# LiJiangnanBit/path_optimizer

Measured on AMD Instinct MI355X. Metric: QP paths/sec at N=200 pts, batch=4096; ADMM iters to 1e-4, higher is better.
Workload: dtype f64

## Files before the change

path_optimizer_amd/csrc/po_capi.cpp:

```cpp
#include <hip/hip_runtime.h>

#include <chrono>
#include <cmath>
#include <cstdint>
#include <cstdio>
#include <algorithm>
#include <cstdlib>
#include <cstring>
#include <limits>
#include <mutex>
#include <new>
#include <string>
#include <thread>
#include <vector>

#include "../../include/po_hip.h"
#include "po_device.hpp"
#include "po_handle.hpp"
#include "po_launch.hpp"
#include "po_map.hpp"
#include "po_smooth.hpp"

namespace {
thread_local std::string g_hip_err;
// ... 204 lines not shown
        HIP_TRY(hipMemcpy(&c, static_cast<int *>(h->nw_idx_buf.p) + h->nw_last_B, sizeof(int), hipMemcpyDeviceToHost));
        *value = c;
        return PO_OK;
    }
    if (k == "newton_list_ok") {
        *value = -1;
        if (!h->nw_idx_buf.p || h->nw_last_B <= 0) return PO_OK;
        HIP_TRY(hipSetDevice(h->device));
        HIP_TRY(hipStreamSynchronize(h->stream));
        const int B = h->nw_last_B;
        std::vector<int> kl(2 * (size_t)B + 1);
        HIP_TRY(hipMemcpy(kl.data(), h->nw_idx_buf.p, sizeof(int) * kl.size(), hipMemcpyDeviceToHost));
        const int *keys = kl.data(), *list = kl.data() + B;
        const int n = list[0];
        int parked = 0;
        for (int b = 0; b < B; ++b) parked += keys[b] >= 0;
        bool ok = n == parked;
        std::vector<char> seen((size_t)B, 0);
        for (int i = 0; ok && i < n; ++i) {
            const int b = list[1 + i];
            ok = b >= 0 && b < B && keys[b] >= 0 && !seen[(size_t)b];
            if (ok) seen[(size_t)b] = 1;
            if (ok && i > 0) { const int a = list[i]; ok = keys[a] > keys[b] || (keys[a] == keys[b] && a < b); }
        }
        *value = ok ? 1 : 0;
        return PO_OK;
    }
    return PO_ERR_INVALID;
}

int po_set_stream(po_handle h, void *hip_stream) {
    if (!h) return PO_ERR_INVALID;
    Lock g(h->mu);
    h->stream = hip_stream ? static_cast<hipStream_t>(hip_stream) : h->own_stream.s;
    return PO_OK;
}

static int make_dev_params(const po_handle_s *h, int form, int keep, po::DevParams *D) {
    const po_params &p = h->params;
    D->d1 = p.d[0]; D->d2 = p.d[1]; D->d3 = p.d[2]; D->d4 = p.d[3];
    if (form == PO_K) {
        D->w_dev = p.k_w_dev; D->w_c = p.k_w_curv; D->w_cr = p.k_w_curv_rate; D->w_s1 = p.w_slack; D->w_s2 = 0; D->w_u = 0; D->w_su = 0;
    } else {
        D->w_dev = p.w_dev; D->w_c = p.w_curv; D->w_cr = p.w_curv_rate; D->w_s1 = p.w_slack;
        D->w_s2 = (form == PO_KPC) ? p.w_k_slack : 0.0;
        D->w_u = keep * p.w_curv_rate;
        D->w_su = (form == PO_KPC) ? p.w_kp_slack * keep : 0.0;
    }
    D->margin = p.margin;
    D->kmax = std::tan(p.max_steer) / p.wheel_base;
    D->max_steer = p.max_steer;
    D->wheel_base = p.wheel_base;
    D->sigma = p.sigma; D->alpha = p.alpha; D->rho0 = p.rho0; D->eps_abs = p.eps_abs; D->eps_rel = p.eps_rel;
    D->eps_pinf = p.eps_prim_inf; D->adapt_tol = p.adapt_tol;
    D->max_iter = p.max_iter; D->check_every = p.check_every; D->adapt_every = p.adapt_every;
    D->end_heading = p.constraint_end_heading;
    D->polish = p.polish; D->pol_delta = p.polish_delta > 0 ? p.polish_delta : 1e-6; D->pol_refine = p.polish_refine_iter < 0 ? 0 : p.polish_refine_iter;
    D->refine = p.refine; D->ref_eps = p.refine_eps; D->ref_rounds = p.refine_rounds;
    D->ref_extra = (p.refine && p.refine_extra_rounds > 0) ? p.refine_extra_rounds : 0;
    D->ref_nw_rho = p.refine_newton_rho > 0 ? std::min(p.refine_newton_rho, po::kRhoMax) : 100.0;
    D->ref_nw_rho_eq = p.refine_newton_rho_eq > 0 ? std::min(p.refine_newton_rho_eq, 1e8) : 1e4;
    D->ref_nw_rho_max = p.refine_newton_rho_max > 0 ? std::min(p.refine_newton_rho_max, po::kRhoMax) : 1e5;
    D->ref_nw_rho_eq_max = p.refine_newton_rho_eq_max > 0 ? std::min(p.refine_newton_rho_eq_max, 1e8) : (p.refine_newton_rho_eq_max < 0 ? 1e6 : 0.0);
    D->ref_ls_tol = p.refine_ls_tol > 0 ? p.refine_ls_tol : 1e-4;
    D->ref_nw_final = p.refine_newton_final; D->ref_nw_esc = p.refine_newton_escalate; D->ref_nw_slice = 0; D->ref_ls_max = p.refine_ls_max > 0 ? p.refine_ls_max : 30; D->ref_nw_max = p.refine_newton_max > 0 ? p.refine_newton_max : 300;
    return PO_OK;
}

static int validate(const po_batch_in *in, int *n, int *m, int *C) {
    if (!in) return PO_ERR_INVALID;
    if (in->B < 0) return PO_ERR_INVALID;
    int rc = po_problem_dims(in->formulation, in->N, in->keep, n, m, C);
    if (rc) return rc;
    if (!in->ref_x || !in->ref_y || !in->ref_z || !in->ref_k || !in->ref_s || !in->bounds || !in->x0 || !in->goal_z) return PO_ERR_INVALID;
    if (in->formulation == PO_KPC && (!in->max_k || !in->max_kp)) return PO_ERR_INVALID;
    if (po_lds_bytes(in->formulation, in->N, *C, in->keep) > 160 * 1024) return PO_ERR_UNSUPPORTED;
    return PO_OK;
}

static void fill_dev_batch(const po_handle_s *h, po::DevBatch *D, const po_batch_in *in, const po_batch_out *out, int n, int m, int C) PO_REQUIRES(h->mu) {
    D->B = in->B; D->N = in->N; D->keep = in->keep; D->C = C;
    D->ref_x = in->ref_x; D->ref_y = in->ref_y; D->ref_z = in->ref_z; D->ref_k = in->ref_k; D->ref_s = in->ref_s;
    D->bounds = in->bounds; D->x0 = in->x0; D->goal_z = in->goal_z; D->max_k = in->max_k; D->max_kp = in->max_kp;
    D->n_points = in->n_points;
    D->order = in->order;
    D->out_states = out ? out->states : nullptr;
    D->out_info = out ? out->info : nullptr;
    D->out_x = out ? out->x : nullptr;
    D->dbg_cycles = nullptr;
    D->only_deferred = 0;
    D->perm_bits = 0;
    if (!h->env_identity && in->B > 8)
        while ((1 << D->perm_bits) < in->B) ++D->perm_bits;
    D->scale = nullptr;
    D->pol_state = nullptr; D->pol_stride = 0;
    D->round = 0;
    D->fb_list = nullptr;
    D->nw_phase = 0; D->nw_state = nullptr; D->nw_stride = 0; D->nw_keys = nullptr; D->nw_list = nullptr;
    D->nw_follows = 0;
    D->fixed_len = (h->fixed_length && !in->n_points && po_has_fixed_length(in->formulation, in->N, C, in->keep)) ? 1 : 0;
    D->n = n; D->m = m;
}

int po_solve_batch_device(po_handle h, const po_batch_in *in, const po_batch_out *out) {
    if (!h || !out || !out->states || !out->info) return PO_ERR_INVALID;
    int n, m, C;
    int rc = validate(in, &n, &m, &C);
    if (rc) return rc;
    if (in->B == 0) return PO_OK;
    Lock g(h->mu);
    HIP_TRY(hipSetDevice(h->device));
    h->timed_host = false;
    po::DevParams P;
    make_dev_params(h, in->formulation, in->keep, &P);
    po::DevBatch D;
    fill_dev_batch(h, &D, in, out, n, m, C);
    const bool dbg = h->env_cycles;
    if (dbg) {
        if ((rc = h->dbg_buf.ensure(sizeof(long long) * 16 * (size_t)in->B))) return rc;
        D.dbg_cycles = static_cast<long long *>(h->dbg_buf.p);
        HIP_TRY(hipMemsetAsync(D.dbg_cycles, 0, sizeof(long long) * 16 * (size_t)in->B, h->stream));
    }
    if ((rc = h->scale_buf.ensure(sizeof(double) * 64 * (size_t)in->B))) return rc;
    D.scale = static_cast<double *>(h->scale_buf.p);
    h->fixed_used = D.fixed_len;
    bool polish = false;
    if (h->params.polish || h->params.refine) {
        const int sd = po_polish_state_doubles(in->formulation, in->N, C, in->keep);
        if (sd > 0) {
            if ((rc = h->pol_buf.ensure(sizeof(double) * (size_t)sd * (size_t)in->B))) return rc;
            D.pol_state = static_cast<double *>(h->pol_buf.p);
            D.pol_stride = sd;
            polish = h->params.polish && po_has_polish_kernel(in->formulation, in->N, C, in->keep);
        }
    }
    const int rounds_total = (h->params.refine_rounds > 1 ? h->params.refine_rounds : 1) + P.ref_extra;
    const bool split = h->params.refine == 2 && D.pol_state != nullptr && rounds_total < 32;
    if (split && ((rc = h->fb_buf.ensure(sizeof(int) * ((size_t)in->B + 1))) || (rc = h->fb_host.ensure(64)))) return rc;
    int pd = 0;
    if (split) {
        const bool slice_auto = in->B >= 2 * h->wave_slots && po_shape_threads(in->formulation, in->N, C, in->keep) == 64;
        pd = (h->nw_slice > 0 && (slice_auto || h->nw_slice_forced)) ? po_newton_park_doubles(in->formulation, in->N, C, in->keep) : 0;
        if (pd > 0 && (h->nw_state_buf.ensure(sizeof(double) * (size_t)pd * (size_t)in->B) || h->nw_idx_buf.ensure(sizeof(int) * (2 * (size_t)in->B + 1)))) {
            (void)hipGetLastError();
            h->nw_state_buf.release();
            pd = 0;
        }
        h->nw_last_B = pd > 0 ? in->B : 0;
    }
    HIP_TRY(hipEventRecord(h->ev0, h->stream));
    h->timed_phases = false;
    HIP_TRY(po_launch_scale(in->formulation, &D, &P, h->params.scaling, static_cast<double *>(h->scale_buf.p), pd > 0 ? static_cast<int *>(h->nw_idx_buf.p) : nullptr,
                            split ? static_cast<int *>(h->fb_buf.p) : nullptr, h->stream));
    if (split) {
        po::DevParams P1 = P;
        for (int r = 1; r < (h->params.refine_rounds > 1 ? h->params.refine_rounds : 1); ++r) { P1.eps_abs *= 10.0; P1.eps_rel *= 10.0; }
        D.nw_follows = 1;
        HIP_TRY(po_launch_solve(in->formulation, &D, &P1, h->stream, nullptr));
        D.nw_follows = 0;
        HIP_TRY(hipEventRecord(h->evp[0], h->stream));
        D.fb_list = static_cast<int *>(h->fb_buf.p);
        if (pd > 0) {
            D.nw_state = static_cast<double *>(h->nw_state_buf.p); D.nw_stride = pd;
            D.nw_keys = static_cast<int *>(h->nw_idx_buf.p); D.nw_list = D.nw_keys + in->B;
            P.ref_nw_slice = h->nw_slice;
            D.nw_phase = 1;
            HIP_TRY(po_launch_newton(in->formulation, &D, &P, h->stream));
            HIP_TRY(po_launch_nw_sort(D.nw_keys, in->B, D.nw_list, h->stream));
            D.nw_phase = 2;
            HIP_TRY(po_launch_newton(in->formulation, &D, &P, h->stream));
            D.nw_phase = 0;
        } else {
            HIP_TRY(po_launch_newton(in->formulation, &D, &P, h->stream));
        }
        HIP_TRY(hipEventRecord(h->evp[1], h->stream));
        h->timed_phases = true;
        bool need_fb = true;
        hipStreamCaptureStatus cap_st = hipStreamCaptureStatusNone;
        const bool capturing = hipStreamIsCapturing(h->stream, &cap_st) == hipSuccess && cap_st != hipStreamCaptureStatusNone;
        if (h->params.refine_chain != 3 && !capturing) {
            volatile int *cnt = static_cast<volatile int *>(h->fb_host.p);
            *cnt = -1;
            HIP_TRY(hipMemcpyAsync(const_cast<int *>(cnt), D.fb_list, sizeof(int), hipMemcpyDeviceToHost, h->stream));
            const auto ts0 = std::chrono::steady_clock::now();
            unsigned spins = 0;
            while (*cnt == -1) {
                if ((++spins & 1023u) == 0 && std::chrono::steady_clock::now() - ts0 > std::chrono::milliseconds(20)) { HIP_TRY(hipStreamSynchronize(h->stream)); break; }
#if defined(__x86_64__) || defined(__i386__)
                __builtin_ia32_pause();
#else
                std::this_thread::yield();
#endif
            }
            need_fb = *cnt != 0;
        }
        if (need_fb) HIP_TRY(po_launch_newton_fallback(in->formulation, &D, &P, h->stream));
    } else {
        HIP_TRY(po_launch_solve(in->formulation, &D, &P, h->stream, nullptr));
    }
    if (split) HIP_TRY(po_launch_finalize_status(D.out_info, in->B, h->stream));
    if (polish) HIP_TRY(po_launch_polish(in->formulation, &D, &P, h->stream));
    {
        const int no_refine = h->params.refine == 2 && !split, no_polish = h->params.polish && !polish;
        if (no_refine || no_polish) HIP_TRY(po_launch_mark_unavailable(D.out_info, in->B, no_refine, no_polish, h->stream));
    }
    HIP_TRY(hipEventRecord(h->ev1, h->stream));
    h->timed = true;
    if (dbg) {
        long long c4[16];
        HIP_TRY(hipStreamSynchronize(h->stream));
        HIP_TRY(hipMemcpy(c4, D.dbg_cycles, sizeof(c4), hipMemcpyDeviceToHost));
        {
            std::vector<long long> all(16 * (size_t)in->B);
            HIP_TRY(hipMemcpy(all.data(), D.dbg_cycles, sizeof(long long) * all.size(), hipMemcpyDeviceToHost));
            long long nf = 0, nb = 0;
            double worst = 0;
            for (int b = 0; b < in->B; ++b) {
                nf += all[16 * (size_t)b + 13]; nb += all[16 * (size_t)b + 14];
                double w; std::memcpy(&w, &all[16 * (size_t)b + 15], sizeof(w)); worst = std::fmax(worst, w);
            }
            std::fprintf(stderr, "[po] batch of %d (form %d, N %d, keep %d): %lld scan factorisations, %lld fell back to the sequential chain; worst relative disagreement scan vs recursion %.3e\n", in->B, in->formulation, in->N, in->keep, nf, nb, worst);
        }
        std::fprintf(stderr, "[po] path0 cycles: rhs %lld solve %lld update %lld over %lld iterations | solve phases F1 %lld F2 %lld F3B1 %lld B2 %lld B3 %lld | first factorisation: blocks %lld chain %lld | uniform row classes %lld | scan factorisations %lld, fell back to the sequential chain %lld\n",
                     c4[0], c4[1], c4[2], c4[3], c4[4], c4[5], c4[6], c4[7], c4[8], c4[10], c4[11], c4[12], c4[13], c4[14]);
    }
    return PO_OK;
}

int po_solve_batch(po_handle h, const po_batch_in *in, const po_batch_out *out) {
    if (!h || !out || !out->states || !out->info) return PO_ERR_INVALID;
    int n, m, C;
    int rc = validate(in, &n, &m, &C);
    if (rc) return rc;
    if (in->B == 0) return PO_OK;
    HIP_TRY(hipSetDevice(h->device));
    const size_t B = in->B, N = in->N;
    const bool kpc = in->formulation == PO_KPC;
    const size_t per_pt = 13 + (kpc ? 2 : 0);
    if (in->n_points)
        for (size_t b = 0; b < B; ++b)
            if (in->n_points[b] < 2 || in->n_points[b] > in->N) return PO_ERR_INVALID;
    if (in->order) {
        std::vector<char> seen(B, 0);
        for (size_t b = 0; b < B; ++b) {
            const int v = in->order[b];
            if (v < 0 || (size_t)v >= B || seen[(size_t)v]) return PO_ERR_INVALID;
            seen[(size_t)v] = 1;
        }
    }
    const size_t in_bytes = sizeof(double) * (B * N * per_pt + B * 4 + 2 * ((B + 1) / 2 + 1));
    const size_t out_bytes = sizeof(double) * (B * N * 5 + (out->x ? B * (size_t)n : 0)) + sizeof(po_info) * B;
    Lock call(h->call_mu);
    hipStream_t st;
    int nthr;
    {
        Lock g(h->mu);
        if ((rc = h->in_buf.ensure(in_bytes)) || (rc = h->out_buf.ensure(out_bytes)) || (rc = h->pin_in.ensure(in_bytes)) || (rc = h->pin_out.ensure(out_bytes))) return rc;
        st = h->stream;
        nthr = h->host_threads > 0 ? h->host_threads : (int)std::min(8u, std::max(1u, std::thread::hardware_concurrency()));
    }
    double *d = static_cast<double *>(h->in_buf.p);
    char *pin = static_cast<char *>(h->pin_in.p);
    po_batch_in din = *in;
    std::vector<CopySeg> segs;
    size_t o = 0;
    auto up = [&](const double *src, size_t cnt, const double **dst) {
        *dst = d + o;
        segs.push_back({pin + o * sizeof(double), reinterpret_cast<const char *>(src), cnt * sizeof(double)});
        o += cnt;
    };
    up(in->ref_x, B * N, &din.ref_x); up(in->ref_y, B * N, &din.ref_y); up(in->ref_z, B * N, &din.ref_z); up(in->ref_k, B * N, &din.ref_k); up(in->ref_s, B * N, &din.ref_s);
    up(in->bounds, B * N * 8, &din.bounds); up(in->x0, B * 3, &din.x0); up(in->goal_z, B, &din.goal_z);
    if (kpc) { up(in->max_k, B * N, &din.max_k); up(in->max_kp, B * N, &din.max_kp); }
    size_t used = o * sizeof(double);
    if (in->n_points) {
        segs.push_back({pin + o * sizeof(double), reinterpret_cast<const char *>(in->n_points), sizeof(int) * B});
        din.n_points = reinterpret_cast<const int *>(d + o);
        used = o * sizeof(double) + sizeof(int) * B;
    }
    if (in->order) {
        const size_t oo = o * sizeof(double) + sizeof(int) * ((B + 1) / 2) * 2;
        segs.push_back({pin + oo, reinterpret_cast<const char *>(in->order), sizeof(int) * B});
        din.order = reinterpret_cast<const int *>(reinterpret_cast<char *>(d) + oo);
        used = oo + sizeof(int) * B;
    }
    double pack_ms, unpack_ms;
    HIP_TRY(hipEventRecord(h->evh[0], st));
    {
        const auto t0 = std::chrono::steady_clock::now();
        const size_t kSlice = (size_t)32 << 20;
        for (size_t lo = 0; lo < used; lo += kSlice) {
            const size_t hi = std::min(used, lo + kSlice);
            std::vector<CopySeg> cur;
            for (const CopySeg &sg : segs) {
                const size_t s0 = (size_t)(sg.dst - pin), s1 = s0 + sg.bytes;
                const size_t a0 = std::max(s0, lo), a1 = std::min(s1, hi);
                if (a0 < a1) cur.push_back({pin + a0, sg.src + (a0 - s0), a1 - a0});
            }
            parallel_copy(cur, nthr);
            HIP_TRY(hipMemcpyAsync(reinterpret_cast<char *>(d) + lo, pin + lo, hi - lo, hipMemcpyHostToDevice, st));
        }
        pack_ms = std::chrono::duration<double, std::milli>(std::chrono::steady_clock::now() - t0).count();
    }
    HIP_TRY(hipEventRecord(h->evh[1], st));
    po_batch_out dout;
    char *ob = static_cast<char *>(h->out_buf.p);
    dout.states = reinterpret_cast<double *>(ob);
    dout.x = out->x ? dout.states + B * N * 5 : nullptr;
    dout.info = reinterpret_cast<po_info *>(ob + sizeof(double) * (B * N * 5 + (out->x ? B * (size_t)n : 0)));
    rc = po_solve_batch_device(h, &din, &dout);
    if (rc) return rc;
    char *pout = static_cast<char *>(h->pin_out.p);
    HIP_TRY(hipMemcpyAsync(pout, ob, out_bytes, hipMemcpyDeviceToHost, st));
    HIP_TRY(hipEventRecord(h->evh[2], st));
    HIP_TRY(hipStreamSynchronize(st));
    {
        const auto t0 = std::chrono::steady_clock::now();
        std::vector<CopySeg> us;
        us.push_back({reinterpret_cast<char *>(out->states), pout, sizeof(double) * B * N * 5});
        if (out->x) us.push_back({reinterpret_cast<char *>(out->x), pout + sizeof(double) * B * N * 5, sizeof(double) * B * (size_t)n});
        us.push_back({reinterpret_cast<char *>(out->info), pout + sizeof(double) * (B * N * 5 + (out->x ? B * (size_t)n : 0)), sizeof(po_info) * B});
        parallel_copy(us, nthr);
        unpack_ms = std::chrono::duration<double, std::milli>(std::chrono::steady_clock::now() - t0).count();
    }
    Lock g(h->mu);
    h->host_pack_ms = pack_ms; h->host_unpack_ms = unpack_ms;
    h->timed_host = true;
    return PO_OK;
}

int po_last_phase_ms(po_handle h, float *ms8) {
    if (!h || !ms8) return PO_ERR_INVALID;
    Lock g(h->mu);
    if (!h->timed) return PO_ERR_INVALID;
    for (int i = 0; i < 8; ++i) ms8[i] = 0.0f;
    HIP_TRY(hipEventSynchronize(h->ev1));
    HIP_TRY(hipEventElapsedTime(&ms8[1], h->ev0, h->ev1));
    if (h->timed_host) {
        HIP_TRY(hipEventSynchronize(h->evh[2]));
        HIP_TRY(hipEventElapsedTime(&ms8[0], h->evh[0], h->evh[1]));
        HIP_TRY(hipEventElapsedTime(&ms8[2], h->ev1, h->evh[2]));
        ms8[3] = (float)h->host_pack_ms; ms8[4] = (float)h->host_unpack_ms;
    }
    if (h->timed_phases) {
        HIP_TRY(hipEventElapsedTime(&ms8[5], h->ev0, h->evp[0]));
        HIP_TRY(hipEventElapsedTime(&ms8[6], h->evp[0], h->evp[1]));
        HIP_TRY(hipEventElapsedTime(&ms8[7], h->evp[1], h->ev1));
    }
    return PO_OK;
}

int po_assemble_batch(po_handle h, const po_batch_in *in, double *l, double *u, double *dyn) {
    if (!h || !l || !u || !dyn) return PO_ERR_INVALID;
    if (in && in->n_points) return PO_ERR_INVALID;
    int n, m, C;
    int rc = validate(in, &n, &m, &C);
    if (rc) return rc;
    if (in->B == 0) return PO_OK;
    const size_t B = in->B, N = in->N;
    const bool kpc = in->formulation == PO_KPC;
    Stage S;
    const Slot<double> rx = S.in(in->ref_x, B * N), ry = S.in(in->ref_y, B * N), rz = S.in(in->ref_z, B * N), rk = S.in(in->ref_k, B * N), rs = S.in(in->ref_s, B * N);
    const Slot<double> bd = S.in(in->bounds, B * N * 8), x0 = S.in(in->x0, B * 3), gz = S.in(in->goal_z, B);
    const Slot<double> mk = S.in(kpc ? in->max_k : nullptr, B * N), mkp = S.in(kpc ? in->max_kp : nullptr, B * N);
    const size_t out_from = (S.bytes() + 15) & ~(size_t)15;
    const Slot<double> dl = S.out(l, B * (size_t)m), du = S.out(u, B * (size_t)m), dd = S.out(dyn, B * (N - 1) * 3);
    return staged_call(h, S, &po_handle_s::asm_buf, false, [&]() -> int {
        Lock g(h->mu);
        po_batch_in din = *in;
        din.ref_x = rx; din.ref_y = ry; din.ref_z = rz; din.ref_k = rk; din.ref_s = rs; din.bounds = bd; din.x0 = x0; din.goal_z = gz;
        if (kpc) { din.max_k = mk; din.max_kp = mkp; }
        HIP_TRY(hipMemsetAsync(dl, 0, S.bytes() - out_from, h->stream));
        po::DevParams P;
        make_dev_params(h, in->formulation, in->keep, &P);
        po::DevBatch D;
        fill_dev_batch(h, &D, &din, nullptr, n, m, C);
        HIP_TRY(po_launch_assemble(in->formulation, &D, &P, dl, du, dd, h->stream));
        return PO_OK;
    });
}

int po_scaling_batch(po_handle h, const po_batch_in *in, double *out) {
    if (!h || !out) return PO_ERR_INVALID;
    if (in && in->n_points) return PO_ERR_INVALID;
    int n, m, C;
    int rc = validate(in, &n, &m, &C);
    if (rc) return rc;
    if (in->B == 0) return PO_OK;
    const size_t B = in->B, N = in->N;
    Stage S;
    const Slot<double> rs = S.in(in->ref_s, B * N), sc = S.out(out, 64 * B);
    return staged_call(h, S, &po_handle_s::asm_buf, false, [&]() -> int {
        Lock g(h->mu);
        po_batch_in din = *in;
        din.ref_s = rs;
        po::DevParams P;
        make_dev_params(h, in->formulation, in->keep, &P);
        po::DevBatch D;
        fill_dev_batch(h, &D, &din, nullptr, n, m, C);
        HIP_TRY(po_launch_scale(in->formulation, &D, &P, h->params.scaling, sc, nullptr, nullptr, h->stream));
        return PO_OK;
    });
}

int po_last_kernel_ms(po_handle h, float *ms) {
    if (!h || !ms) return PO_ERR_INVALID;
    Lock g(h->mu);
    if (!h->timed) return PO_ERR_INVALID;
    HIP_TRY(hipEventSynchronize(h->ev1));
    HIP_TRY(hipEventElapsedTime(ms, h->ev0, h->ev1));
    return PO_OK;
}

static po::DevCar make_car(const po_params &p) {
    po::DevCar c{};
    const double width = p.car_width, back = p.car_length / 2.0 - p.rear_axle_to_center, front = p.car_length / 2.0 + p.rear_axle_to_center;
    const double length = front + back;
    c.bx = (front - back) / 2.0;
    c.br = std::sqrt((length / 2) * (length / 2) + (width / 2) * (width / 2));
    const double shift = width / 4.0, small_r = std::sqrt(2 * (shift * shift));
    const double large_r = std::sqrt(width * width + ((length - width) / 2.0) * ((length - width) / 2.0)) / 2;
    const double px[4] = {-back + shift, -back + shift, front - shift, front - shift};
    const double py[4] = {-width / 2.0 + shift, width / 2.0 - shift, -width / 2.0 + shift, width / 2.0 - shift};
    for (int i = 0; i < 4; ++i) { c.cx[i] = px[i]; c.cy[i] = py[i]; c.cr[i] = small_r; }
    c.cx[4] = c.bx + (length - width) / 4; c.cy[4] = 0; c.cr[4] = large_r;
    c.cx[5] = c.bx - (length - width) / 4; c.cy[5] = 0; c.cr[5] = large_r;
    c.enable = p.enable_collision_check;
    return c;
}

static void publish_stack(po_handle h, int M, int sx, int sy, double res, double px, double py, bool layer_pos) PO_REQUIRES(h->mu) {
    const bool keep = h->maps.M == M && h->maps.layer_of;
    po::DevMaps s{};
    s.d = static_cast<const float *>(h->map_buf.p); s.sx = sx; s.sy = sy; s.res = res; s.px = px; s.py = py;
    s.M = M; s.stride = (size_t)sx * (size_t)sy;
    s.pos = layer_pos ? static_cast<const double *>(h->map_pos_buf.p) : nullptr;
    s.layer_of = keep ? static_cast<const int *>(h->map_assign_buf.p) : nullptr;
    s.n_assign = keep ? h->maps.n_assign : 0;
    h->maps = s;
}
static int install_layers(po_handle h, int M, const po_map *map, const double *pos_xy) PO_REQUIRES(h->mu) {
    HIP_TRY(hipSetDevice(h->device));
    const size_t bytes = sizeof(float) * (size_t)M * (size_t)map->size_x * (size_t)map->size_y;
    if (bytes > h->map_buf.cap) h->maps.d = nullptr;
    if (int rc = grow_after_sync(h, h->map_buf, bytes)) return rc;
    if (pos_xy) {
        if (int rc = grow_after_sync(h, h->map_pos_buf, sizeof(double) * 2 * (size_t)M)) return rc;
        HIP_TRY(hipMemcpyAsync(h->map_pos_buf.p, pos_xy, sizeof(double) * 2 * (size_t)M, hipMemcpyHostToDevice, h->stream));
    }
    HIP_TRY(hipMemcpyAsync(h->map_buf.p, map->distance, bytes, hipMemcpyHostToDevice, h->stream));
    HIP_TRY(hipStreamSynchronize(h->stream));
    publish_stack(h, M, map->size_x, map->size_y, map->resolution, map->pos_x, map->pos_y, pos_xy != nullptr);
    return PO_OK;
}

int po_set_map(po_handle h, const po_map *map) {
    if (!h || !map || !map->distance || map->size_x < 1 || map->size_y < 1 || !(map->resolution > 0)) return PO_ERR_INVALID;
    Lock g(h->mu);
    return install_layers(h, 1, map, nullptr);
}

int po_set_map_stack(po_handle h, int M, const po_map *layers, const double *pos_xy) {
    if (!h || M < 1 || !layers || !layers->distance || layers->size_x < 1 || layers->size_y < 1 || !(layers->resolution > 0)) return PO_ERR_INVALID;
    if (layers->size_x > po_edt_max_side() || layers->size_y > po_edt_max_side() || M > po_edt_max_images()) return PO_ERR_UNSUPPORTED;
    Lock call(h->call_mu);
    Lock g(h->mu);
    return install_layers(h, M, layers, pos_xy);
}

int po_set_map_assignment_device(po_handle h, int n, const int *layer_of) {
    if (!h || n < 0) return PO_ERR_INVALID;
    Lock g(h->mu);
    if (n == 0 || !layer_of) {
        h->maps.layer_of = nullptr; h->maps.n_assign = 0;
        return PO_OK;
    }
    if (!h->maps.d) return PO_ERR_INVALID;
    HIP_TRY(hipSetDevice(h->device));
    if (int rc = grow_after_sync(h, h->map_assign_buf, sizeof(int) * (size_t)n)) return rc;
    HIP_TRY(hipMemcpyAsync(h->map_assign_buf.p, layer_of, sizeof(int) * (size_t)n, hipMemcpyDeviceToDevice, h->stream));
    h->maps.layer_of = static_cast<const int *>(h->map_assign_buf.p); h->maps.n_assign = n;
    return PO_OK;
}

int po_set_map_assignment(po_handle h, int n, const int *layer_of) {
    if (!h || n < 0) return PO_ERR_INVALID;
    Lock call(h->call_mu);
    Lock g(h->mu);
    if (n == 0 || !layer_of) {
        h->maps.layer_of = nullptr; h->maps.n_assign = 0;
        return PO_OK;
    }
    if (!h->maps.d) return PO_ERR_INVALID;
    for (int b = 0; b < n; ++b)
        if (layer_of[b] < 0 || layer_of[b] >= h->maps.M) return PO_ERR_INVALID;
    HIP_TRY(hipSetDevice(h->device));
    if (int rc = grow_after_sync(h, h->map_assign_buf, sizeof(int) * (size_t)n)) {
        h->maps.layer_of = nullptr; h->maps.n_assign = 0;
        return rc;
    }
    HIP_TRY(hipMemcpyAsync(h->map_assign_buf.p, layer_of, sizeof(int) * (size_t)n, hipMemcpyHostToDevice, h->stream));
    HIP_TRY(hipStreamSynchronize(h->stream));
    h->maps.layer_of = static_cast<const int *>(h->map_assign_buf.p); h->maps.n_assign = n;
    return PO_OK;
}

static int check_occupancy(po_handle h, int M, const po_occupancy *occ) {
    if (!h || M < 1 || !occ || !occ->cells || occ->size_x < 1 || occ->size_y < 1 || !(occ->resolution > 0)) return PO_ERR_INVALID;
    if (occ->size_x > po_edt_max_side() || occ->size_y > po_edt_max_side() || M > po_edt_max_images()) return PO_ERR_UNSUPPORTED;
    return PO_OK;
}

int po_distance_map_batch_device(po_handle h, int M, const po_occupancy *occ, float *distance) {
    if (int rc = check_occupancy(h, M, occ)) return rc;
    if (!distance) return PO_ERR_INVALID;
    Lock g(h->mu);
    HIP_TRY(hipSetDevice(h->device));
    if (int rc = grow_after_sync(h, h->edt_buf, po_edt_scratch_bytes(M, occ->size_x, occ->size_y))) return rc;
    HIP_TRY(po_launch_edt(occ->cells, M, occ->size_x, occ->size_y, (float)occ->resolution, h->edt_buf.p, distance, h->stream));
    return PO_OK;
}

int po_distance_map_batch(po_handle h, int M, const po_occupancy *occ, float *distance) {
    if (int rc = check_occupancy(h, M, occ)) return rc;
    if (!distance) return PO_ERR_INVALID;
    const size_t cells = (size_t)M * (size_t)occ->size_x * (size_t)occ->size_y;
    Stage S;
    const Slot<float> d_dist = S.out(distance, cells);
    const Slot<unsigned char> d_cells = S.in(occ->cells, cells);
    return staged_call(h, S, &po_handle_s::edt_io, true, [&] {
        po_occupancy dev = *occ;
        dev.cells = d_cells;
        return po_distance_map_batch_device(h, M, &dev, d_dist);
    });
}

static int stack_from_images(po_handle h, int M, const unsigned char *cells, int sx, int sy, double res, double px, double py, const double *pos_xy)
    PO_REQUIRES(h->mu) {
    const size_t stack_bytes = sizeof(float) * (size_t)M * (size_t)sx * (size_t)sy;
    if (stack_bytes > h->map_buf.cap) h->maps.d = nullptr;
    if (int rc = grow_after_sync(h, h->map_buf, stack_bytes)) return rc;
    if (int rc = grow_after_sync(h, h->edt_buf, po_edt_scratch_bytes(M, sx, sy))) return rc;
    if (pos_xy) {
        if (int rc = grow_after_sync(h, h->map_pos_buf, sizeof(double) * 2 * (size_t)M)) return rc;
        HIP_TRY(hipMemcpyAsync(h->map_pos_buf.p, pos_xy, sizeof(double) * 2 * (size_t)M, hipMemcpyDeviceToDevice, h->stream));
    }
    HIP_TRY(po_launch_edt(cells, M, sx, sy, (float)res, h->edt_buf.p, static_cast<float *>(h->map_buf.p), h->stream));
    publish_stack(h, M, sx, sy, res, px, py, pos_xy != nullptr);
// ... 996 lines not shown
```

path_optimizer_amd/csrc/po_kernels.hip:

```cpp
#include "po_solve_common.hpp"

namespace po {

template <int F> __global__ __launch_bounds__(64) void assemble_kernel(DevBatch in, DevParams P, double *l, double *u, double *dyn) {
    using T = FormTraits<F>;
    extern __shared__ double smem[];
    const int b = blockIdx.x;
    Ctx<F> cx(P, in, smem, b);
    const int N = cx.N, C = cx.C;
    double *lb = l + (size_t)b * in.m, *ub = u + (size_t)b * in.m;
    for (int j = cx.lane; j < N; j += 64) {
        const StageIn si = cx.stage_in(j);
        AsmFn<F> fn{lb, ub, j, N, C, 0};
        local_rows<F>(si, P, fn);
        if (T::NEND && si.last) { fn.kind = 1; end_rows<F>(si, P, fn); }
        double bin[3];
        if (j == 0) cx.init_bounds(bin);
        else {
            const Dyn<F> d = cx.dyn(j - 1);
#pragma unroll
            for (int r = 0; r < T::NDYN; ++r) bin[r] = d.b[r];
            double *dd = dyn + ((size_t)b * (N - 1) + (j - 1)) * 3;
            if constexpr (F == F_K) { dd[0] = d.f[0][0]; dd[1] = d.f[1][1]; dd[2] = d.f[0][2]; }
            else { dd[0] = d.f[0][1]; dd[1] = d.f[1][0]; dd[2] = d.beta[2]; }
// ... 39 lines not shown
const Object kObjects[] = {PO_SOLVE_OBJECTS(PO_X)};
#undef PO_X
struct Resolved { Shape s; size_t lds; int group; bool fixed; };
hipError_t resolve(int form, const DevBatch *in, Resolved *r) {
    r->lds = 0;
    if (!resolve_shape(form, in->N, in->C, in->keep, &r->s)) return hipErrorInvalidValue;
    r->lds = lds_of(form, in->N, in->C, r->s);
    r->group = group_of(form, r->s);
#ifdef PO_DEV_HEADLINE
    if (form == F_KP && r->group) r->group = ~0;
#endif
    r->fixed = in->fixed_len && in->n_points == nullptr && is_fixed_shape(form, in->N, in->C, in->keep, r->s);
    return r->lds > 160 * 1024 ? hipErrorInvalidValue : hipSuccess;
}
hipError_t call(int form, int kind, int launch, const Resolved &r, const DevBatch *in, const DevParams *P, hipStream_t st) {
    for (const Object &o : kObjects)
        if (o.form == form && o.kind == kind && (o.groups & r.group) && o.entry) return o.entry(launch, r.s, r.lds, in, P, st);
    return hipErrorNotSupported;
}
}
}
extern "C" hipError_t po_launch_solve(int form, const po::DevBatch *in, const po::DevParams *P, hipStream_t st, size_t *lds_out) {
    using namespace po;
    Resolved r;
    hipError_t e = resolve(form, in, &r);
    if (lds_out && r.lds) *lds_out = r.lds;
    if (e != hipSuccess) return e;
    const bool uni = form == F_K ? has_uni_variant<F_K>(r.s) : has_uni_variant<F_KP>(r.s);
    DevBatch copy = *in;
    copy.only_deferred = 0;
    if (uni && (e = call(form, r.fixed ? kObjFixUni : kObjUni, kLaunchSolve, r, &copy, P, st)) != hipSuccess) return e;
    copy.only_deferred = uni ? 1 : 0;
    return call(form, kObjGen, kLaunchSolve, r, &copy, P, st);
}
extern "C" hipError_t po_launch_finalize_status(po_info *info, int B, hipStream_t st) {
    hipLaunchKernelGGL(po::finalize_status_kernel, dim3((B + 255) / 256), dim3(256), 0, st, info, B);
    return hipGetLastError();
}

static hipError_t launch_two_level(int form, int launch, const po::DevBatch *in, const po::DevParams *P, hipStream_t st) {
    using namespace po;
    Resolved r;
    const hipError_t e = resolve(form, in, &r);
    if (!r.lds || !r.s.two) return hipErrorInvalidValue;
    if (launch == kLaunchPolish && !has_polish_kernel(r.s)) return hipSuccess;
    if (e != hipSuccess) return e;
    const int kind = (launch == kLaunchNewton && r.fixed) ? (in->nw_phase == 2 ? kObjFixNewton2 : kObjFixNewton1) : (launch == kLaunchPolish ? kObjGen : kObjNewton);
    return call(form, kind, launch, r, in, P, st);
}
extern "C" hipError_t po_launch_newton(int form, const po::DevBatch *in, const po::DevParams *P, hipStream_t st) { return launch_two_level(form, po::kLaunchNewton, in, P, st); }
extern "C" hipError_t po_launch_newton_fallback(int form, const po::DevBatch *in, const po::DevParams *P, hipStream_t st) { return launch_two_level(form, po::kLaunchFallback, in, P, st); }
extern "C" hipError_t po_launch_polish(int form, const po::DevBatch *in, const po::DevParams *P, hipStream_t st) { return launch_two_level(form, po::kLaunchPolish, in, P, st); }
namespace po {
constexpr int kNwSortThreads = 256;
__global__ __launch_bounds__(kNwSortThreads) void nw_sort_kernel(const int *keys, int B, int *list) {
    __shared__ int cnt[kNwKeys][kNwSortThreads + 1];
    __shared__ int rowbase[kNwKeys];
    const int t = threadIdx.x, per = (B + kNwSortThreads - 1) / kNwSortThreads, lo = t * per, hi = min(B, lo + per);
    constexpr int kCache = 16;
    int kc[kCache];
#pragma unroll
    for (int i = 0; i < kCache; ++i) kc[i] = (lo + i < hi) ? keys[lo + i] : -1;
#pragma unroll
    for (int k = 0; k < kNwKeys; ++k) cnt[k][t] = 0;
#pragma unroll
    for (int i = 0; i < kCache; ++i)
        if (kc[i] >= 0) cnt[kc[i] < kNwKeys ? kc[i] : kNwKeys - 1][t] += 1;
    for (int b = lo + kCache; b < hi; ++b) {
        const int k = keys[b];
        if (k >= 0) cnt[k < kNwKeys ? k : kNwKeys - 1][t] += 1;
    }
    __syncthreads();
    {
        constexpr int kPerLane = kNwSortThreads / 64, kWaves = kNwSortThreads / 64;
        const int lane = t & 63, wv = t >> 6;
        for (int k = wv; k < kNwKeys; k += kWaves) {
            int v[kPerLane], sum = 0;
#pragma unroll
            for (int i = 0; i < kPerLane; ++i) { v[i] = cnt[k][lane * kPerLane + i]; sum += v[i]; }
            int incl = sum;
#pragma unroll
            for (int d = 1; d < 64; d <<= 1) { const int o = __shfl_up(incl, d, 64); if (lane >= d) incl += o; }
            int run = incl - sum;
#pragma unroll
            for (int i = 0; i < kPerLane; ++i) { cnt[k][lane * kPerLane + i] = run; run += v[i]; }
            if (lane == 63) cnt[k][kNwSortThreads] = incl;
        }
    }
    __syncthreads();
    if (t < kNwKeys) {
        int run = 0;
        for (int j = kNwKeys - 1; j > t; --j) run += cnt[j][kNwSortThreads];
        rowbase[t] = run;
        if (t == 0) list[0] = run + cnt[0][kNwSortThreads];
    }
    __syncthreads();
    auto place = [&](int b, int k) {
        const int kk = k < kNwKeys ? k : kNwKeys - 1;
        const int pos = rowbase[kk] + cnt[kk][t];
        cnt[kk][t] += 1;
        list[1 + pos] = b;
    };
#pragma unroll
    for (int i = 0; i < kCache; ++i)
        if (kc[i] >= 0) place(lo + i, kc[i]);
    for (int b = lo + kCache; b < hi; ++b) {
        const int k = keys[b];
        if (k >= 0) place(b, k);
    }
}

}
extern "C" hipError_t po_launch_nw_sort(const int *keys, int B, int *list, hipStream_t st) {
    hipLaunchKernelGGL(po::nw_sort_kernel, dim3(1), dim3(po::kNwSortThreads), 0, st, keys, B, list);
    return hipGetLastError();
}
namespace po {
namespace {
template <int F, bool TWO, int SPL, int NT, int NWX> struct RowSizes { static constexpr int state = 0, park = 0; };
template <int F, int SPL, int NT, int NWX> struct RowSizes<F, true, SPL, NT, NWX> {
    static constexpr int state = Fast<F, SPL, NT, true, NWX>::kStateDoubles * NT, park = Fast<F, SPL, NT, true, NWX>::kParkDoubles * NT + kNwParkScalars;
};
int row_doubles(int form, int N, int C, int keep, bool park) {
    Shape s;
    if (!resolve_shape(form, N, form == F_K ? 0 : C, keep, &s)) return 0;
#define PO_X(F_, TWO_, SPL_, NT_, NWX_, G_) if (form == F_ && is_shape(s, TWO_, SPL_, NT_, NWX_)) return park ? RowSizes<F_, TWO_, SPL_, NT_, NWX_>::park : RowSizes<F_, TWO_, SPL_, NT_, NWX_>::state;
    PO_SHAPE_ROWS(PO_X)
#undef PO_X
    return 0;
}
}
}
extern "C" int po_polish_state_doubles(int form, int N, int C, int keep) { return po::row_doubles(form, N, C, keep, false); }
extern "C" int po_newton_park_doubles(int form, int N, int C, int keep) { return po::row_doubles(form, N, C, keep, true); }
extern "C" int po_has_fixed_length(int form, int N, int C, int keep) {
    po::Shape s;
    if (!po::resolve_shape(form, N, C, keep, &s) || !po::is_fixed_shape(form, N, C, keep, s) || po::lds_of(form, N, C, s) > 160 * 1024) return 0;
#define PO_X(N_) if (N == N_) return 1;
    PO_FIXED_LIST(PO_X)
#undef PO_X
    return 0;
}
extern "C" int po_shape_threads(int form, int N, int C, int keep) {
    po::Shape s;
    return po::resolve_shape(form, N, form == po::F_K ? 0 : C, keep, &s) ? s.nt : 0;
}
extern "C" int po_has_polish_kernel(int form, int N, int C, int keep) {
    po::Shape s;
    return po::resolve_shape(form, N, form == po::F_K ? 0 : C, keep, &s) && po::has_polish_kernel(s);
}

extern "C" hipError_t po_launch_scale(int form, const po::DevBatch *in, const po::DevParams *P, int passes, double *sc, int *nw_keys, int *fb_count, hipStream_t st) {
    using namespace po;
    const int bs = 64, gs = (in->B + bs - 1) / bs;
    if (form == F_KP) hipLaunchKernelGGL(scale_kernel<F_KP>, dim3(gs), dim3(bs), 0, st, *in, *P, passes, sc, nw_keys, fb_count);
    else if (form == F_KPC) hipLaunchKernelGGL(scale_kernel<F_KPC>, dim3(gs), dim3(bs), 0, st, *in, *P, passes, sc, nw_keys, fb_count);
    else hipLaunchKernelGGL(scale_kernel<F_K>, dim3(gs), dim3(bs), 0, st, *in, *P, passes, sc, nw_keys, fb_count);
    return hipGetLastError();
}

extern "C" hipError_t po_launch_assemble(int form, const po::DevBatch *in, const po::DevParams *P, double *l, double *u, double *dyn, hipStream_t st) {
    using namespace po;
    if (form == F_KP) hipLaunchKernelGGL(assemble_kernel<F_KP>, dim3(in->B), dim3(64), 0, st, *in, *P, l, u, dyn);
    else if (form == F_KPC) hipLaunchKernelGGL(assemble_kernel<F_KPC>, dim3(in->B), dim3(64), 0, st, *in, *P, l, u, dyn);
    else hipLaunchKernelGGL(assemble_kernel<F_K>, dim3(in->B), dim3(64), 0, st, *in, *P, l, u, dyn);
    return hipGetLastError();
}

extern "C" size_t po_lds_bytes(int form, int N, int C, int keep) {
    using namespace po;
    Shape s;
    if (!resolve_shape(form, N, C, keep, &s)) return (size_t)1 << 30;
    return lds_of(form, N, C, s);
}
```

path_optimizer_amd/csrc/po_scale.hpp:

```cpp
#pragma once
#include "po_device.hpp"

namespace po {

constexpr int kNVC = 8;
constexpr int kNRC = 24;
constexpr int kScStride = 64;
constexpr int kScW = 0, kScE = 24, kScSig = 48, kScCD = 56, kScC = 63;
constexpr int kKEndRow = 11, kKEndVar = 6, kScAlt = 12;
constexpr double kMinScaling = 1e-4, kMaxScaling = 1e4;

struct ClassModel {
    int nr;
    double Pmax[kNVC], cnt[kNVC];
    double a[kNRC][kNVC];
    int tgt[kNRC];
};

struct PatFn {
    ClassModel *M;
    int base;
    template <int MASK, class TL, class TU> __host__ __device__ void row(int r, double c0, double c1, double c2, double c3, double c4, TL, TU) {
        double *a = M->a[base + r];
        a[0] = c0; a[1] = c1; a[2] = c2; a[3] = c3; a[4] = c4;
    }
};
struct PatCtlFn {
    ClassModel *M;
    int base;
    template <int MASK, class TL, class TU> __host__ __device__ void row(int r, double, double, double c2, double c3, double, TL, TU) {
        double *a = M->a[base + r];
        a[5] = c2; a[6] = c3;
    }
};

__device__ inline double limit_scaling(double v) {
    v = v < kMinScaling ? 1.0 : v;
    return v > kMaxScaling ? kMaxScaling : v;
}

template <int F> __device__ void class_scaling(const DevParams &P, int N, int keep, int C, double ds_nom, int passes, double *out ) {
#pragma clang fp contract(off)
    using T = FormTraits<F>;
    ClassModel M;
    M.nr = T::NLOC + T::NDYN + T::NCTL + T::NEND;
    for (int r = 0; r < kNRC; ++r) { M.tgt[r] = -1; for (int v = 0; v < kNVC; ++v) M.a[r][v] = 0; }
    StageIn s;
    for (int c = 0; c < 4; ++c) { s.lb[c] = -1; s.ub[c] = 1; }
    s.maxk = 0; s.elo = -kInf; s.ehi = kInf; s.j = 0; s.N = N; s.last = 0;
    PatFn pf{&M, 0};
    local_rows<F>(s, P, pf);
    const Dyn<F> d = make_dyn<F>(0.0, ds_nom, P);
    for (int r = 0; r < T::NDYN; ++r) {
        double *a = M.a[T::NLOC + r];
        a[0] = d.f[r][0]; a[1] = d.f[r][1]; a[2] = d.f[r][2]; a[5] = d.beta[r];
        M.tgt[T::NLOC + r] = dyn_tau<F>(r);
    }
    if constexpr (T::NCTL > 0) { PatCtlFn cf{&M, T::NLOC + T::NDYN}; ctl_rows<F>(0.0, cf); }
    if constexpr (T::NEND > 0) { PatFn ef{&M, T::NLOC + T::NDYN + T::NCTL}; end_rows<F>(s, P, ef); }
    if constexpr (F == F_K) {
        static_assert(T::NLOC + T::NDYN == kKEndRow && kScAlt + T::NLOC <= 24, "K end classes");
        M.a[kKEndRow][kKEndVar] = M.a[2][2];
        M.a[T::NLOC + 0][kKEndVar] = M.a[T::NLOC + 0][2];
        M.nr = kKEndRow + 1;
    }
    for (int v = 0; v < kNVC; ++v) { M.Pmax[v] = 0; M.cnt[v] = 0; }
    M.Pmax[0] = P.w_dev; M.Pmax[2] = (F == F_K) ? P.w_c + 2 * P.w_cr : P.w_c; M.Pmax[3] = P.w_s1;
    M.cnt[0] = N; M.cnt[1] = N; M.cnt[2] = N; M.cnt[3] = N;
    if constexpr (F == F_K) { M.Pmax[kKEndVar] = P.w_c + P.w_cr; M.cnt[kKEndVar] = N - 1 < 2 ? N - 1 : 2; M.cnt[2] = N - 1 - M.cnt[kKEndVar]; }
    if constexpr (F == F_KP) { M.Pmax[5] = P.w_u; M.cnt[5] = C; M.Pmax[7] = P.w_s1; M.cnt[7] = N; }
    if constexpr (F == F_KPC) { M.Pmax[4] = P.w_s2; M.cnt[4] = N; M.Pmax[5] = P.w_u; M.cnt[5] = C; M.Pmax[6] = P.w_su; M.cnt[6] = C; M.cnt[7] = N - C; }
    double Dv[kNVC], Er[kNRC], c = 1.0, ntot = 0;
    for (int v = 0; v < kNVC; ++v) { Dv[v] = 1.0; ntot += M.cnt[v]; }
    for (int r = 0; r < kNRC; ++r) Er[r] = 1.0;
    for (int pass = 0; pass < passes; ++pass) {
        double cn[kNVC], rn[kNRC];
        for (int v = 0; v < kNVC; ++v) cn[v] = fabs(c * M.Pmax[v] * Dv[v] * Dv[v]);
        for (int r = 0; r < M.nr; ++r) {
            double rmax = 0;
            for (int v = 0; v < kNVC; ++v) {
                const double a = fabs(Er[r] * M.a[r][v] * Dv[v]);
                if (a > rmax) rmax = a;
                if (a > cn[v]) cn[v] = a;
            }
            if (M.tgt[r] >= 0) {
                const double a = fabs(Er[r] * Dv[M.tgt[r]]);
                if (a > rmax) rmax = a;
                if (a > cn[M.tgt[r]]) cn[M.tgt[r]] = a;
            }
            rn[r] = rmax;
        }
        for (int v = 0; v < kNVC; ++v) Dv[v] *= 1.0 / sqrt(limit_scaling(cn[v]));
        for (int r = 0; r < M.nr; ++r) Er[r] *= 1.0 / sqrt(limit_scaling(rn[r]));
        double mean = 0;
        for (int v = 0; v < kNVC; ++v) mean += M.cnt[v] * fabs(c * M.Pmax[v] * Dv[v] * Dv[v]);
        mean /= ntot;
        double ct = mean > 1.0 ? mean : 1.0;
        ct = 1.0 / limit_scaling(ct);
        c *= ct;
    }
    for (int i = 0; i < kScStride; ++i) out[i] = 0;
    for (int r = 0; r < kNRC; ++r) { out[kScW + r] = Er[r] * Er[r] / c; out[kScE + r] = Er[r]; }
    for (int v = 0; v < 7; ++v) { out[kScSig + v] = P.sigma / (c * Dv[v] * Dv[v]); out[kScCD + v] = c * Dv[v]; }
    if constexpr (F == F_K) {
        for (int r = 0; r < T::NLOC; ++r) { out[kScW + kScAlt + r] = out[kScW + (r == 2 ? kKEndRow : r)]; out[kScE + kScAlt + r] = out[kScE + (r == 2 ? kKEndRow : r)]; }
    }
    out[kScC] = c;
}

template <int F> __global__ void scale_kernel(DevBatch in, DevParams P, int passes, double *sc, int *nw_keys, int *fb_count) {
    const int b = blockIdx.x * blockDim.x + threadIdx.x;
    if (b >= in.B) return;
    if (nw_keys) nw_keys[b] = -1;
    if (fb_count && b == 0) *fb_count = 0;
    const double *s = in.ref_s + (size_t)b * in.N;
    int N = in.N, C = in.C;
    if (in.n_points) { N = in.n_points[b]; N = N < 2 ? 2 : (N > in.N ? in.N : N); C = (F == F_K) ? N - 1 : (N + in.keep - 2) / in.keep; }
    double ds_nom = 0;
    for (int i = 1; i < N && i < 10; ++i) ds_nom = fmax(ds_nom, __dsub_rn(s[i], s[i - 1]));
    class_scaling<F>(P, N, in.keep, C, ds_nom, passes, sc + (size_t)b * kScStride);
}

}
```

Baseline: 1.215 million.

## Parallelize per-path scaling across 32 lanes and skip finalize when no fallback

The scaling kernel previously ran one thread per path, looping serially over all row and variable classes. It now assigns 32 lanes per path, one per row class, and computes column maxima with xor-shuffle reductions, broadcasting factors through shuffles. The finalize-status launch is now skipped unless the Newton fallback ran, which removes one kernel launch in the common case. The scaling batch API also accepts per-path point counts. Risks include more redundant per-lane model construction, possible output slots left unwritten (kScStride is no longer zeroed), and the finalize skip changing status handling.

```diff
diff --git a/path_optimizer_amd/csrc/po_capi.cpp b/path_optimizer_amd/csrc/po_capi.cpp
--- a/path_optimizer_amd/csrc/po_capi.cpp
+++ b/path_optimizer_amd/csrc/po_capi.cpp
@@ -380,6 +380,7 @@
     h->timed_phases = false;
     HIP_TRY(po_launch_scale(in->formulation, &D, &P, h->params.scaling, static_cast<double *>(h->scale_buf.p), pd > 0 ? static_cast<int *>(h->nw_idx_buf.p) : nullptr,
                             split ? static_cast<int *>(h->fb_buf.p) : nullptr, h->stream));
+    bool need_finalize = false;
     if (split) {
         po::DevParams P1 = P;
         for (int r = 1; r < (h->params.refine_rounds > 1 ? h->params.refine_rounds : 1); ++r) { P1.eps_abs *= 10.0; P1.eps_rel *= 10.0; }
@@ -423,10 +424,11 @@
             need_fb = *cnt != 0;
         }
         if (need_fb) HIP_TRY(po_launch_newton_fallback(in->formulation, &D, &P, h->stream));
+        need_finalize = need_fb;
     } else {
         HIP_TRY(po_launch_solve(in->formulation, &D, &P, h->stream, nullptr));
     }
-    if (split) HIP_TRY(po_launch_finalize_status(D.out_info, in->B, h->stream));
+    if (split && need_finalize) HIP_TRY(po_launch_finalize_status(D.out_info, in->B, h->stream));
     if (polish) HIP_TRY(po_launch_polish(in->formulation, &D, &P, h->stream));
     {
         const int no_refine = h->params.refine == 2 && !split, no_polish = h->params.polish && !polish;
@@ -610,7 +612,6 @@
 
 int po_scaling_batch(po_handle h, const po_batch_in *in, double *out) {
     if (!h || !out) return PO_ERR_INVALID;
-    if (in && in->n_points) return PO_ERR_INVALID;
     int n, m, C;
     int rc = validate(in, &n, &m, &C);
     if (rc) return rc;
@@ -618,10 +619,12 @@
     const size_t B = in->B, N = in->N;
     Stage S;
     const Slot<double> rs = S.in(in->ref_s, B * N), sc = S.out(out, 64 * B);
+    const Slot<int> np = S.in(in->n_points, B);
     return staged_call(h, S, &po_handle_s::asm_buf, false, [&]() -> int {
         Lock g(h->mu);
         po_batch_in din = *in;
         din.ref_s = rs;
+        din.n_points = np;
         po::DevParams P;
         make_dev_params(h, in->formulation, in->keep, &P);
         po::DevBatch D;
diff --git a/path_optimizer_amd/csrc/po_kernels.hip b/path_optimizer_amd/csrc/po_kernels.hip
--- a/path_optimizer_amd/csrc/po_kernels.hip
+++ b/path_optimizer_amd/csrc/po_kernels.hip
@@ -215,7 +215,7 @@
 
 extern "C" hipError_t po_launch_scale(int form, const po::DevBatch *in, const po::DevParams *P, int passes, double *sc, int *nw_keys, int *fb_count, hipStream_t st) {
     using namespace po;
-    const int bs = 64, gs = (in->B + bs - 1) / bs;
+    const int bs = kScBlock, gs = (int)(((size_t)in->B * kScLanes + bs - 1) / bs);
     if (form == F_KP) hipLaunchKernelGGL(scale_kernel<F_KP>, dim3(gs), dim3(bs), 0, st, *in, *P, passes, sc, nw_keys, fb_count);
     else if (form == F_KPC) hipLaunchKernelGGL(scale_kernel<F_KPC>, dim3(gs), dim3(bs), 0, st, *in, *P, passes, sc, nw_keys, fb_count);
     else hipLaunchKernelGGL(scale_kernel<F_K>, dim3(gs), dim3(bs), 0, st, *in, *P, passes, sc, nw_keys, fb_count);
diff --git a/path_optimizer_amd/csrc/po_scale.hpp b/path_optimizer_amd/csrc/po_scale.hpp
--- a/path_optimizer_amd/csrc/po_scale.hpp
+++ b/path_optimizer_amd/csrc/po_scale.hpp
@@ -39,10 +39,9 @@
     return v > kMaxScaling ? kMaxScaling : v;
 }
 
-template <int F> __device__ void class_scaling(const DevParams &P, int N, int keep, int C, double ds_nom, int passes, double *out ) {
+template <int F> __device__ __forceinline__ void class_model(const DevParams &P, int N, int C, double ds_nom, ClassModel &M) {
 #pragma clang fp contract(off)
     using T = FormTraits<F>;
-    ClassModel M;
     M.nr = T::NLOC + T::NDYN + T::NCTL + T::NEND;
     for (int r = 0; r < kNRC; ++r) { M.tgt[r] = -1; for (int v = 0; v < kNVC; ++v) M.a[r][v] = 0; }
     StageIn s;
@@ -70,55 +69,104 @@
     if constexpr (F == F_K) { M.Pmax[kKEndVar] = P.w_c + P.w_cr; M.cnt[kKEndVar] = N - 1 < 2 ? N - 1 : 2; M.cnt[2] = N - 1 - M.cnt[kKEndVar]; }
     if constexpr (F == F_KP) { M.Pmax[5] = P.w_u; M.cnt[5] = C; M.Pmax[7] = P.w_s1; M.cnt[7] = N; }
     if constexpr (F == F_KPC) { M.Pmax[4] = P.w_s2; M.cnt[4] = N; M.Pmax[5] = P.w_u; M.cnt[5] = C; M.Pmax[6] = P.w_su; M.cnt[6] = C; M.cnt[7] = N - C; }
-    double Dv[kNVC], Er[kNRC], c = 1.0, ntot = 0;
+}
+
+constexpr int kScLanes = 32, kScBlock = 256;
+static_assert(kNRC <= kScLanes && kNVC == 8 && kScBlock % kScLanes == 0 && 64 % kScLanes == 0, "scale_kernel: a lane per row class, groups inside a wave");
+__device__ __forceinline__ double sc_max(double m, double a) { return a > m ? a : m; }
+
+template <int F> __global__ __launch_bounds__(kScBlock) void scale_kernel(DevBatch in, DevParams P, int passes, double *sc, int *nw_keys, int *fb_count) {
+#pragma clang fp contract(off)
+    using T = FormTraits<F>;
+    const int t = blockIdx.x * kScBlock + threadIdx.x, b = t / kScLanes, l = t % kScLanes;
+    if (b >= in.B) return;
+    if (l == 0) {
+        if (nw_keys) nw_keys[b] = -1;
+        if (fb_count && b == 0) *fb_count = 0;
+    }
+    const double *s = in.ref_s + (size_t)b * in.N;
+    int N = in.N, C = in.C;
+    if (in.n_points) { N = in.n_points[b]; N = N < 2 ? 2 : (N > in.N ? in.N : N); C = (F == F_K) ? N - 1 : (N + in.keep - 2) / in.keep; }
+    double sv[10];
+#pragma unroll
+    for (int i = 0; i < 10; ++i) sv[i] = s[i < N ? i : N - 1];
+    double ds_nom = 0;
+#pragma unroll
+    for (int i = 1; i < 10; ++i)
+        if (i < N) ds_nom = fmax(ds_nom, __dsub_rn(sv[i], sv[i - 1]));
+    ClassModel M;
+    class_model<F>(P, N, C, ds_nom, M);
+    const bool row = l < M.nr;
+    const int vc = l & 7;
+    double a[kNVC], Pv = 0;
+    int tgt = -1;
+#pragma unroll
+    for (int v = 0; v < kNVC; ++v) { a[v] = 0; Pv = v == vc ? M.Pmax[v] : Pv; }
+#pragma unroll
+    for (int r = 0; r < kNRC; ++r) {
+        tgt = r == l ? M.tgt[r] : tgt;
+#pragma unroll
+        for (int v = 0; v < kNVC; ++v) a[v] = r == l ? M.a[r][v] : a[v];
+    }
+    double Dv[kNVC], Dc = 1.0, Er = 1.0, c = 1.0, ntot = 0;
+#pragma unroll
     for (int v = 0; v < kNVC; ++v) { Dv[v] = 1.0; ntot += M.cnt[v]; }
-    for (int r = 0; r < kNRC; ++r) Er[r] = 1.0;
     for (int pass = 0; pass < passes; ++pass) {
-        double cn[kNVC], rn[kNRC];
-        for (int v = 0; v < kNVC; ++v) cn[v] = fabs(c * M.Pmax[v] * Dv[v] * Dv[v]);
-        for (int r = 0; r < M.nr; ++r) {
-            double rmax = 0;
-            for (int v = 0; v < kNVC; ++v) {
-                const double a = fabs(Er[r] * M.a[r][v] * Dv[v]);
-                if (a > rmax) rmax = a;
-                if (a > cn[v]) cn[v] = a;
-            }
-            if (M.tgt[r] >= 0) {
-                const double a = fabs(Er[r] * Dv[M.tgt[r]]);
-                if (a > rmax) rmax = a;
-                if (a > cn[M.tgt[r]]) cn[M.tgt[r]] = a;
-            }
-            rn[r] = rmax;
+        double col[kNVC], rmax = 0;
+#pragma unroll
+        for (int v = 0; v < kNVC; ++v) {
+            col[v] = sc_max(0.0, fabs(Er * a[v] * Dv[v]));
+            rmax = sc_max(rmax, col[v]);
         }
-        for (int v = 0; v < kNVC; ++v) Dv[v] *= 1.0 / sqrt(limit_scaling(cn[v]));
-        for (int r = 0; r < M.nr; ++r) Er[r] *= 1.0 / sqrt(limit_scaling(rn[r]));
+        {
+            double dt = 0;
+#pragma unroll
+            for (int v = 0; v < kNVC; ++v) dt = v == tgt ? Dv[v] : dt;
+            const double at = tgt >= 0 ? sc_max(0.0, fabs(Er * dt)) : 0.0;
+            rmax = sc_max(rmax, at);
+#pragma unroll
+            for (int v = 0; v < kNVC; ++v) col[v] = v == tgt ? sc_max(col[v], at) : col[v];
+        }
+        double c4[4], c2[2], cm;
+#pragma unroll
+        for (int i = 0; i < 4; ++i) {
+            const bool hi = (l & 1) != 0;
+            c4[i] = sc_max(hi ? col[2 * i + 1] : col[2 * i], __shfl_xor(hi ? col[2 * i] : col[2 * i + 1], 1, kScLanes));
+        }
+#pragma unroll
+        for (int i = 0; i < 2; ++i) {
+            const bool hi = (l & 2) != 0;
+            c2[i] = sc_max(hi ? c4[2 * i + 1] : c4[2 * i], __shfl_xor(hi ? c4[2 * i] : c4[2 * i + 1], 2, kScLanes));
+        }
+        {
+            const bool hi = (l & 4) != 0;
+            cm = sc_max(hi ? c2[1] : c2[0], __shfl_xor(hi ? c2[0] : c2[1], 4, kScLanes));
+        }
+        cm = sc_max(cm, __shfl_xor(cm, 8, kScLanes));
+        cm = sc_max(cm, __shfl_xor(cm, 16, kScLanes));
+        const double cn = sc_max(fabs(c * Pv * Dc * Dc), cm);
+        const double fc = 1.0 / sqrt(limit_scaling(cn));
+        Dc *= fc;
+#pragma unroll
+        for (int v = 0; v < kNVC; ++v) Dv[v] *= __shfl(fc, v, kScLanes);
+        if (row) Er *= 1.0 / sqrt(limit_scaling(rmax));
         double mean = 0;
+#pragma unroll
         for (int v = 0; v < kNVC; ++v) mean += M.cnt[v] * fabs(c * M.Pmax[v] * Dv[v] * Dv[v]);
         mean /= ntot;
         double ct = mean > 1.0 ? mean : 1.0;
         ct = 1.0 / limit_scaling(ct);
         c *= ct;
     }
-    for (int i = 0; i < kScStride; ++i) out[i] = 0;
-    for (int r = 0; r < kNRC; ++r) { out[kScW + r] = Er[r] * Er[r] / c; out[kScE + r] = Er[r]; }
-    for (int v = 0; v < 7; ++v) { out[kScSig + v] = P.sigma / (c * Dv[v] * Dv[v]); out[kScCD + v] = c * Dv[v]; }
+    double *out = sc + (size_t)b * kScStride;
+    double w = Er * Er / c, e = Er;
     if constexpr (F == F_K) {
-        for (int r = 0; r < T::NLOC; ++r) { out[kScW + kScAlt + r] = out[kScW + (r == 2 ? kKEndRow : r)]; out[kScE + kScAlt + r] = out[kScE + (r == 2 ? kKEndRow : r)]; }
+        const int r = l - kScAlt, src = (r >= 0 && r < T::NLOC) ? (r == 2 ? kKEndRow : r) : l;
+        w = __shfl(w, src, kScLanes); e = __shfl(e, src, kScLanes);
     }
-    out[kScC] = c;
-}
-
-template <int F> __global__ void scale_kernel(DevBatch in, DevParams P, int passes, double *sc, int *nw_keys, int *fb_count) {
-    const int b = blockIdx.x * blockDim.x + threadIdx.x;
-    if (b >= in.B) return;
-    if (nw_keys) nw_keys[b] = -1;
-    if (fb_count && b == 0) *fb_count = 0;
-    const double *s = in.ref_s + (size_t)b * in.N;
-    int N = in.N, C = in.C;
-    if (in.n_points) { N = in.n_points[b]; N = N < 2 ? 2 : (N > in.N ? in.N : N); C = (F == F_K) ? N - 1 : (N + in.keep - 2) / in.keep; }
-    double ds_nom = 0;
-    for (int i = 1; i < N && i < 10; ++i) ds_nom = fmax(ds_nom, __dsub_rn(s[i], s[i - 1]));
-    class_scaling<F>(P, N, in.keep, C, ds_nom, passes, sc + (size_t)b * kScStride);
+    if (l < kNRC) { out[kScW + l] = w; out[kScE + l] = e; }
+    if (l < 7) { out[kScSig + l] = P.sigma / (c * Dc * Dc); out[kScCD + l] = c * Dc; }
+    if (l == 7) { out[kScSig + 7] = 0; out[kScC] = c; }
 }
 
 }
```

After: 1.218 million (median of 6 runs). No clear change (+0.3%).
